# sanowl/CUDA-NT-Xent-MPI-NCCL-SimCLR

Hardware: AMD Instinct MI355X
Metric: NT-Xent fwd+bwd samples/sec, B=4096 d=2048, at 1/2/4/8 MI355X (higher is better)
Workload: dtype bf16

## Files before the change

cuda-nt-xent-mpi-nccl-simclr_amd/csrc/kernels/ntxent_kernels.hip:

```cpp

#include "../include/ntxent/ntxent.h"
#include "device_common.h"
#include "sim_gemm.h"

#include <atomic>
#include <algorithm>
#include <cmath>
#include <cstdio>
#include <cstdlib>
#include <mutex>
#include <string>
#include <type_traits>
#include <vector>
#include <unordered_map>

namespace ntxent {
namespace dev {

template <typename T> __device__ __forceinline__ void load8(const T* p, float (&v)[8]);
template <> __device__ __forceinline__ void load8<float>(const float* p, float (&v)[8]) {
  const f32x4 a = *reinterpret_cast<const f32x4*>(p), b = *reinterpret_cast<const f32x4*>(p + 4);
  v[0] = a[0]; v[1] = a[1]; v[2] = a[2]; v[3] = a[3]; v[4] = b[0]; v[5] = b[1]; v[6] = b[2]; v[7] = b[3];
}
template <typename T> __device__ __forceinline__ void load8_h(const T* p, float (&v)[8]) {
// ... 1457 lines not shown
  NTXENT_HIP_CHECK(hipGetLastError());
}

int dot_slots(const Geometry& g) { return 4 * g.col_tiles; }

void launch_dot_reduce(const float* dotp, float* dot, const Geometry& g, hipStream_t stream) {
  hipLaunchKernelGGL(dev::dot_reduce_kernel, dim3((g.rows_pad + 31) / 32), dim3(256), 0, stream, dotp, dot_slots(g),
                     g.rows_pad, dot);
  NTXENT_HIP_CHECK(hipGetLastError());
}

static bool apply_norm_fuse(dev::SimParams& p, const NormFuse* nf, const Geometry& g) {
  if (nf == nullptr || nf->dh == nullptr || g.dim % 8 != 0) return false;
  p.nh = nf->h;
  p.nh_dt = nf->in == DType::F32 ? 0 : (nf->in == DType::F16 ? 1 : 2);
  p.nd = g.dim;
  p.ninv = nf->inv;
  p.ndot = nf->dot;
  p.ngo = nf->grad_out;
  p.nalpha = (float)(1.0 / ((double)g.global_rows * g.temperature));
  p.ndh = nf->dh;
  p.out_f16 = 1;
  p.accum = 0;
  return true;
}

bool launch_dz(DType comp, const void* sc, const void* zqt_all, const int4* tiles, int ntiles,
               void* slabs, const GemmWorkspace& ws, const Geometry& g, hipStream_t stream, bool out_f16,
               const NormFuse* nf, const Q8Stats* q8, const float* cpos, bool half_c) {
  if (ntiles == 0) return false;
  NTXENT_CHECK(!half_c || dz_half_c_eligible(comp, g, ntiles, ws), "dz: half C not eligible for this launch");
  const bool f8 = comp == DType::FP8;
  NTXENT_CHECK(!f8 || (q8 && q8->mneg2 && q8->lmin && q8->zq && cpos && g.world == 1 && out_f16),
               "dz (fp8 backward): Q8Stats, cpos, world 1 and an fp16 slab required");
  const long long cs = (long long)dtype_size(comp);
  dev::SimParams p = base_params(g);
  if (f8) {
    p.q8_mneg = q8->mneg2;
    p.q8_lmin = q8->lmin;
    p.q8_zq = static_cast<const _Float16*>(q8->zq);
    p.q8_ldz = g.ld_k;
    p.cpos = cpos;
  }
  p.A = coef_tile_operand(sc, g.col_tiles, cs);
  p.B.base = static_cast<const char*>(zqt_all);
  const long long ldt = f8 ? q8_ldt(g) : g.ld_t;
  p.B.ld = ldt * cs;
  p.B.row_tile_stride = (long long)kTile * ldt * cs;
  p.B.kblk = (long long)g.rows_pad * cs;
  p.B.kblk_stride = (long long)g.dim_n * ldt * cs;
  p.tiles = tiles;
  p.kbytes = (long long)g.world * g.rows_pad * cs;
  p.out = static_cast<float*>(slabs);
  p.out_f16 = out_f16 ? 1 : 0;
  p.ldo = g.dim_n;
  p.slab_stride = (long long)g.rows_pad * g.dim_n;
  const int cus = ws.sched_cus > 0 ? std::min(ws.sched_cus, ws.num_cus) : ws.num_cus;
  const int nk = (int)(p.kbytes / kKStepBytes);
  int pieces = fwd_splitk_pieces(ntiles, nk, cus, 1);
  if (pieces < 3 || f8) pieces = 0;
  int grid;
  if (pieces > 0) {
    p.nk = nk;
    p.dp_tiles = 0;
    p.sk_tiles = ntiles;
    p.ipb = (nk + pieces - 1) / pieces;
    p.sk_cnt = static_cast<int*>(ws.ptr);
    p.sk_slabs = reinterpret_cast<float*>(static_cast<char*>(ws.ptr) + sk_counter_bytes(ws.num_cus));
    p.splitk = 1;
    grid = (int)((nk + p.ipb - 1) / p.ipb) * ntiles;
    NTXENT_CHECK(p.kbytes % kKStepBytes == 0 && grid <= ws.num_cus && ws.ptr != nullptr &&
                     ws.bytes >= gemm_workspace_bytes(ntiles, ws.num_cus),
                 "split-K dZ: workspace too small");
  } else {
    grid = apply_schedule(p, ntiles, ws, stream);
  }
  if (half_c)
    NTXENT_CHECK(((pieces == 0 && p.sk_tiles == 0 && p.dp_tiles == ntiles) || (pieces > 0 && p.ipb % 2 == 0)) &&
                     (long long)g.row_tiles * g.col_tiles * kTileElems * cs < (1ll << 31),
                 "dz: half C needs items starting at even K-steps and a C buffer below 2 GiB (32-bit offsets)");
  p.c_half = half_c ? 1 : 0;
  const bool fused = comp != DType::F32 && apply_norm_fuse(p, nf, g);
  if (fused) NTXENT_CHECK(nf->dot != nullptr, "dz: fused normalisation backward without dot");
  if (nf && nf->dot_cnt) {
    NTXENT_CHECK(fused && !f8 && nf->dotp && dz_dot_fold_eligible(comp, g, ntiles, ws),
                 "dz: dot fold needs the fused 16-bit epilogue");
    p.dotp = const_cast<float*>(nf->dotp);
    p.dot_nslot = dot_slots(g);
    p.dot_cnt = pieces == 0 ? nf->dot_cnt : nullptr;
    p.dot_spin = dot_fold_spin();
  }
  dispatch_gemm(comp, [&](auto tc) {
    using Tc = decltype(tc);
    launch_sim_gemm<Tc, dev::kModeDz>(grid, p, stream);
  });
  if (pieces > 0) hipLaunchKernelGGL(dev::sk_dz_reduce_kernel, dim3(ntiles * 64), dim3(256), 0, stream, p);
  NTXENT_HIP_CHECK(hipGetLastError());
  return fused;
}

void launch_dz_view(DType comp, const void* a, long long a_panel_tiles, const void* b, long long b_kblk_cols,
                    long long b_kblk_stride, int k_tiles, const int4* tiles, int ntiles, void* out, bool accum,
                    const GemmWorkspace& ws, const Geometry& g, hipStream_t stream, bool out_f16) {
  NTXENT_CHECK(!(accum && out_f16), "dz_view: fp16 output cannot accumulate");
  if (ntiles == 0 || k_tiles == 0) return;
  NTXENT_CHECK(k_tiles > 0 && a_panel_tiles >= k_tiles, "dz_view: bad K extent");
  const long long cs = (long long)dtype_size(comp);
  dev::SimParams p = base_params(g);
  p.A = coef_tile_operand(a, a_panel_tiles, cs);
  NTXENT_CHECK(b_kblk_cols > 0 && b_kblk_cols % kTile == 0, "dz_view: bad B K block");
  p.B.base = static_cast<const char*>(b);
  p.B.ld = (long long)g.ld_t * cs;
  p.B.row_tile_stride = (long long)kTile * g.ld_t * cs;
  p.B.kblk = b_kblk_cols * cs;
  p.B.kblk_stride = b_kblk_stride * cs;
  p.tiles = tiles;
  p.kbytes = (long long)k_tiles * kTile * cs;
  p.out = static_cast<float*>(out);
  p.ldo = g.dim_n;
  p.slab_stride = (long long)g.rows_pad * g.dim_n;
  p.accum = accum ? 1 : 0;
  p.out_f16 = out_f16 ? 1 : 0;
  const int grid = apply_schedule(p, ntiles, ws, stream);
  dispatch_comp(comp, [&](auto tc) {
    using Tc = decltype(tc);
    launch_sim_gemm<Tc, dev::kModeDz>(grid, p, stream);
  });
  NTXENT_HIP_CHECK(hipGetLastError());
}

void launch_norm_bwd(DType in, const float* slabs, int nslabs, const void* h, const float* inv,
                     const float* grad_out, void* dh, const Geometry& g, hipStream_t stream,
                     const void* xslabs, int nx) {
  const _Float16* xs = static_cast<const _Float16*>(xslabs);
  if (xs == nullptr) nx = 0;
  const float alpha_base = (float)(1.0 / ((double)g.global_rows * g.temperature));
  const long long ss = (long long)g.rows_pad * g.dim_n, ldo = g.dim_n;
  const int nch = (g.dim + 2047) / 2048;
  const bool vec = (g.dim % 8) == 0 && nch <= 4;
  dispatch_comp(in, [&](auto tin) {
    using Tin = decltype(tin);
    const Tin* hp = static_cast<const Tin*>(h);
    Tin* dp = static_cast<Tin*>(dh);
    if (vec && nch == 1)
      hipLaunchKernelGGL((dev::norm_bwd_vec_kernel<Tin, 1>), dim3(g.rows), dim3(256), 0, stream, slabs, nslabs, ss,
                         ldo, hp, inv, grad_out, alpha_base, dp, g.dim, xs, nx);
    else if (vec && nch == 2)
      hipLaunchKernelGGL((dev::norm_bwd_vec_kernel<Tin, 2>), dim3(g.rows), dim3(256), 0, stream, slabs, nslabs, ss,
                         ldo, hp, inv, grad_out, alpha_base, dp, g.dim, xs, nx);
    else if (vec)
      hipLaunchKernelGGL((dev::norm_bwd_vec_kernel<Tin, 4>), dim3(g.rows), dim3(256), 0, stream, slabs, nslabs, ss,
                         ldo, hp, inv, grad_out, alpha_base, dp, g.dim, xs, nx);
    else
      hipLaunchKernelGGL((dev::norm_bwd_kernel<Tin>), dim3(g.rows), dim3(256), 0, stream, slabs, nslabs, ss, ldo,
                         hp, inv, grad_out, alpha_base, dp, g.dim, xs, nx);
  });
  NTXENT_HIP_CHECK(hipGetLastError());
}

const DeviceInfo& device_info(int device) {
  static std::mutex mu;
  static std::unordered_map<int, DeviceInfo> cache;
  std::lock_guard<std::mutex> lock(mu);
  auto it = cache.find(device);
  if (it != cache.end()) return it->second;
  hipDeviceProp_t prop;
// ... 23 lines not shown
```

cuda-nt-xent-mpi-nccl-simclr_amd/csrc/kernels/sim_gemm.h:

```cpp
#pragma once

#include "../include/ntxent/ntxent.h"
#include "device_common.h"

#include <type_traits>

namespace ntxent {
namespace dev {

enum SimMode : int { kModeFwd = 0, kModeCoef = 1, kModeDz = 2 };

constexpr int kStageBytes = 2 * kTile * kKStepBytes;
#ifndef NTXENT_GEMM_DMA_AUX
#define NTXENT_GEMM_DMA_AUX 0
#endif
constexpr int kGemmDmaAux = NTXENT_GEMM_DMA_AUX;
#ifndef NTXENT_TIMING
#define NTXENT_TIMING 0
#endif
constexpr int kTimingItems = 8;
constexpr int kTimingMarks = 8;
__device__ __forceinline__ void store16_wt(void* base, long long off, u32x4 v) {
  const unsigned lo = __builtin_amdgcn_readfirstlane((unsigned)off);
  const unsigned hi = __builtin_amdgcn_readfirstlane((unsigned)((unsigned long long)off >> 32));
// ... 75 lines not shown

__device__ __forceinline__ int sc_unit(int rb, int cb, int lane) { return ((rb >> 4) * 8 + (cb >> 5)) * 64 + lane; }

struct KStream {
  const char* ptr;
  int kin, left;
  int kk;
  __device__ __forceinline__ void init(const char* base, long long k0, const OperandDesc& o, int nk) {
    kin = (int)(k0 % o.kblk);
    ptr = base + (k0 / o.kblk) * o.kblk_stride + kin;
    left = nk - 1;
    kk = (int)(k0 / kKStepBytes);
  }
  __device__ __forceinline__ void advance(const OperandDesc& o) {
    if (left > 0) {
      --left;
      ++kk;
      ptr += kKStepBytes;
      kin += kKStepBytes;
      if (kin == (int)o.kblk) { kin = 0; ptr += o.kblk_stride - o.kblk; }
    }
  }
  __device__ __forceinline__ void skip() {
    if (left > 0) {
      --left;
      ++kk;
    }
  }
  __device__ __forceinline__ void seek(const char* base, long long k0, const OperandDesc& o) {
    kin = (int)(k0 % o.kblk);
    ptr = base + (k0 / o.kblk) * o.kblk_stride + kin;
  }
};

__device__ __forceinline__ int ct_swz(int L) {
  return ((L >> 1) & 1) | ((L & 1) << 1) | (((L >> 3) & 1) << 2) | ((((L >> 1) ^ (L >> 2)) & 1) << 3);
}

__device__ __forceinline__ void dot_slot_store(float* p, float v) { *p = v; }

__device__ __forceinline__ long long ctile_index(const SimParams& p, int mt, int nt) {
  const int cs = p.c_rot ? (nt - p.row_tile0 + p.col_tiles) % p.col_tiles : nt - p.c_tile0;
  return (long long)mt * p.c_ld + cs;
}

template <typename T, int NW, int NMI = 8>
__device__ __forceinline__ void coef_epilogue(f32x4 (&acc)[NMI][4], const int (&rb)[NMI], const int (&cb)[4],
                                              int row_base, int col_base, int mt, int nt, int kind,
                                              lds_char* lds, const SimParams& p, int lane) {
  constexpr int NROWS = NW == 8 ? kTile : NMI * 16;
  constexpr int NCOLS = NW == 8 ? kTile : 64;
#ifndef NTXENT_COEF_SWZ
#define NTXENT_COEF_SWZ 1
#endif
  constexpr bool SWZ = NW == 1 && NTXENT_COEF_SWZ;
  static_assert(!SWZ || (NROWS == 64 && NCOLS == 64), "swizzled C^T staging is for 64 x 64 regions");
  constexpr int S = SWZ ? 128 : NROWS * 2 + 16;
  auto ct_at = [&](int L, int e) { return SWZ ? L * S + (((e >> 2) ^ ct_swz(L)) << 3) : L * S + e * 2; };
  constexpr int NT = NW * 64;
  T* base = reinterpret_cast<T*>(p.cbuf);
  const int col_local0 = (nt * kTile) % p.Rpad;
  const bool fixed = p.fixed_shift != 0;
  const float M = p.y_scale;
  float lcol[4];
  bool cvalid[4];
  int gj[4];
#pragma unroll
  for (int ni = 0; ni < 4; ++ni) {
    const int col_t = cb[ni] + (lane & 15);
    gj[ni] = nt * kTile + col_t;
    const float l = p.lse2[gj[ni]];
    lcol[ni] = fixed ? fast_exp2(M - l) : l;
    cvalid[ni] = (col_local0 + col_t) < p.R;
  }
  T* slot = base + ctile_index(p, mt, nt) * kTileElems;
  T* mirror = nullptr;
  if ((kind == kTileSymOff && !p.c_half) || kind == kTileDiagUp)
    mirror = base + ctile_index(p, nt - p.row_tile0, p.row_tile0 + mt) * kTileElems;
  else if (kind == kTileCross) {
    const int rt = p.Rpad / kTile, W = p.col_tiles / rt, q = nt / rt;
    const int slot = (q - p.row_tile0 / rt - 1 + W) % W;
    mirror = reinterpret_cast<T*>(p.mbuf) + ((long long)(slot * rt + nt % rt) * rt + mt) * kTileElems;
  }
  const int wq = NW == 8 ? ((threadIdx.x >> 6) & 3) : (col_base >> 6);
  float cdot[2][4] = {{0.f, 0.f, 0.f, 0.f}, {0.f, 0.f, 0.f, 0.f}};
  const int r_lo = mt * kTile + row_base, r_hi = r_lo + NROWS;
  const int c_lo = nt * kTile + col_base, c_hi = c_lo + NCOLS;
  auto hits = [&](int a0) { return a0 < c_hi && c_lo < a0 + NROWS; };
  const bool plain = fixed && r_hi <= p.R && col_local0 + col_base + NCOLS <= p.R && !hits(p.own0 + r_lo) &&
                     !hits(p.own0 + r_lo + p.n_half) && !hits(p.own0 + r_lo - p.n_half);
#pragma unroll
  for (int mi = 0; mi < NMI; ++mi) {
    float c[4][4];
    const int row_t0 = rb[mi] + 4 * (lane >> 4);
    const int gi0 = mt * kTile + row_t0;
    const f32x4 lrow4 = *reinterpret_cast<const f32x4*>(p.lse2 + p.own0 + gi0);
    const f32x4 cpos4 = *reinterpret_cast<const f32x4*>(p.cpos + gi0);
    if (plain) {
#pragma unroll
      for (int r = 0; r < 4; ++r) {
        const float lrow = fast_exp2(M - lrow4[r]);
#pragma unroll
        for (int ni = 0; ni < 4; ++ni) c[ni][r] = fast_exp2(acc[mi][ni][r] * p.acc_scale - M) * (lrow + lcol[ni]);
      }
    } else
#pragma unroll
    for (int r = 0; r < 4; ++r) {
      const int gi = gi0 + r;
      const bool rvalid = gi < p.R;
      const float lrow = fixed ? fast_exp2(M - lrow4[r]) : lrow4[r];
      const int gself = p.own0 + gi;
      const int gpos = p.own0 + (gi < p.n_half ? gi + p.n_half : gi - p.n_half);
#pragma unroll
      for (int ni = 0; ni < 4; ++ni) {
        const float y = acc[mi][ni][r] * p.acc_scale;
        float v = fixed ? fast_exp2(y - M) * (lrow + lcol[ni]) : fast_exp2(y - lrow) + fast_exp2(y - lcol[ni]);
        v = (gj[ni] == gpos) ? cpos4[r] : v;
        v = (rvalid && cvalid[ni] && gj[ni] != gself) ? v : 0.0f;
        c[ni][r] = v;
      }
    }
    if (p.dotp) {
#pragma unroll
      for (int r = 0; r < 4; ++r) {
        float d = 0.f;
#pragma unroll
        for (int ni = 0; ni < 4; ++ni) d += to_f32<T>(from_f32<T>(c[ni][r])) * acc[mi][ni][r];
        d = row16_sum(d);
        const int row = mt * kTile + rb[mi] + 4 * (lane >> 4) + r;
        if ((lane & 15) == 0) dot_slot_store(p.dotp + (long long)(nt * 4 + wq) * p.Rpad + row, d);
      }
      const int h2 = NMI == 8 ? (mi >> 2) : 0;
#pragma unroll
      for (int ni = 0; ni < 4; ++ni)
#pragma unroll
        for (int r = 0; r < 4; ++r) cdot[h2][ni] += to_f32<T>(from_f32<T>(c[ni][r])) * acc[mi][ni][r];
    }
#pragma unroll
    for (int ni = 0; ni < 4; ++ni) {
      const int col_t = cb[ni] + (lane & 15);
      if constexpr (sizeof(T) == 2) {
        union { T h[4]; u32x2 u; } pk;
#pragma unroll
        for (int r = 0; r < 4; ++r) pk.h[r] = from_f32<T>(c[ni][r]);
        *reinterpret_cast<__attribute__((address_space(3))) u32x2*>(lds + ct_at(col_t - col_base, row_t0 - row_base)) =
            pk.u;
      } else {
#pragma unroll
        for (int r = 0; r < 4; ++r)
          *reinterpret_cast<float*>(reinterpret_cast<char*>(slot) + ctile_off(row_t0 + r, col_t, 4)) = c[ni][r];
        if (mirror)
          *reinterpret_cast<f32x4*>(reinterpret_cast<char*>(mirror) + ctile_off(col_t, row_t0, 4)) =
              f32x4{c[ni][0], c[ni][1], c[ni][2], c[ni][3]};
      }
    }
  }
  if (p.dotp) {
    if (kind == kTileSymOff || kind == kTileDiagUp) {
      const int wa8 = (threadIdx.x >> 6) >> 2;
#pragma unroll
      for (int h2 = 0; h2 < (NMI == 8 ? 2 : 1); ++h2)
#pragma unroll
        for (int ni = 0; ni < 4; ++ni) {
          const float d = xrow_sum(cdot[h2][ni]);
          const int rq = NMI == 8 ? 2 * h2 + wa8 : (row_base >> 6);
          const int row = (nt - p.row_tile0) * kTile + cb[ni] + (lane & 15);
          if (lane < 16) dot_slot_store(p.dotp + (long long)((p.row_tile0 + mt) * 4 + rq) * p.Rpad + row, d);
        }
    }
  }
  if constexpr (sizeof(T) == 2) {
    __syncthreads();
    const int tid = threadIdx.x, w = tid >> 6;
    if (mirror) {
      constexpr int CPR = NROWS * 2 / 16;
#pragma unroll 4
      for (int q = 0; q < NCOLS * CPR / NT; ++q) {
        const int k = tid + NT * q;
        const int row = k / CPR, c16 = k % CPR;
        u32x4 v;
        if constexpr (SWZ) {
          typedef __attribute__((address_space(3))) const u32x2 lds_u2;
          const u32x2 lo = *(lds_u2*)(lds + ct_at(row, 8 * c16)), hi = *(lds_u2*)(lds + ct_at(row, 8 * c16 + 4));
          v = u32x4{lo[0], lo[1], hi[0], hi[1]};
        } else {
          v = *reinterpret_cast<const __attribute__((address_space(3))) u32x4*>(lds + row * S + c16 * 16);
        }
        *reinterpret_cast<u32x4*>(reinterpret_cast<char*>(mirror) + ctile_off(col_base + row, row_base + 8 * c16, 2)) = v;
      }
    }
    typedef short v4s __attribute__((ext_vector_type(4)));
    constexpr int RB = NROWS / 16;
    constexpr int NBLK = RB * (NCOLS / 32) / NW;
    const int g = lane >> 4, i = lane & 15, q4 = i >> 2, p4 = i & 3;
#pragma unroll 2
    for (int b = 0; b < NBLK; ++b) {
      const int blk = w * NBLK + b;
      const int c0 = (blk % RB) * 16;
      const int r0 = (blk / RB) * 32 + 8 * g;
      const lds_char* a0 = lds + ct_at(r0 + q4, c0 + 4 * p4);
      const lds_char* a1 = lds + ct_at(r0 + q4 + 4, c0 + 4 * p4);
      const v4s lo = __builtin_amdgcn_ds_read_tr16_b64_v4i16((__attribute__((address_space(3))) v4s*)a0);
      const v4s hi = __builtin_amdgcn_ds_read_tr16_b64_v4i16((__attribute__((address_space(3))) v4s*)a1);
      u32x4 u;
      u[0] = (unsigned short)lo[0] | ((unsigned)(unsigned short)lo[1] << 16);
      u[1] = (unsigned short)lo[2] | ((unsigned)(unsigned short)lo[3] << 16);
      u[2] = (unsigned short)hi[0] | ((unsigned)(unsigned short)hi[1] << 16);
      u[3] = (unsigned short)hi[2] | ((unsigned)(unsigned short)hi[3] << 16);
      const int src = ((lane >> 2) + 16 * (lane & 3)) << 2;
      u32x4 v;
#pragma unroll
      for (int k = 0; k < 4; ++k) v[k] = (unsigned)__builtin_amdgcn_ds_bpermute(src, (int)u[k]);
      char* cdst = reinterpret_cast<char*>(slot) +
                   ctile_off(row_base + c0 + (lane >> 2), col_base + (blk / RB) * 32 + 8 * (lane & 3), 2);
#ifndef NTXENT_COEF_STORE
#define NTXENT_COEF_STORE 0
#endif
      if constexpr (NTXENT_COEF_STORE == 1)
        __builtin_nontemporal_store(v, reinterpret_cast<u32x4*>(cdst));
      else if constexpr (NTXENT_COEF_STORE == 2)
        store16_wt(slot, cdst - reinterpret_cast<char*>(slot), v);
      else
        *reinterpret_cast<u32x4*>(cdst) = v;
    }
  }
}

__device__ __forceinline__ unsigned q8_pack4(float x0, float x1, float x2, float x3) {
  const int w = __builtin_amdgcn_cvt_pk_fp8_f32(fminf(x0, 448.f), fminf(x1, 448.f), 0, false);
  return (unsigned)__builtin_amdgcn_cvt_pk_fp8_f32(fminf(x2, 448.f), fminf(x3, 448.f), w, true);
}
__device__ __forceinline__ float q8_dot4(unsigned w, const f32x4& a) {
  typedef float f2 __attribute__((ext_vector_type(2)));
  const f2 lo = __builtin_amdgcn_cvt_pk_f32_fp8((int)w, false), hi = __builtin_amdgcn_cvt_pk_f32_fp8((int)w, true);
  return fmaf(lo[0], a[0], fmaf(lo[1], a[1], fmaf(hi[0], a[2], hi[1] * a[3])));
}

template <typename TS>
__device__ __forceinline__ void coef_epilogue_q8(f32x4 (&acc)[4][4], const int (&rb)[4], const int (&cb)[4],
                                                 int row_base, int col_base, int mt, int nt, int kind, lds_char* lds,
                                                 const SimParams& p, int lane) {
  constexpr int S8 = 80;
  lds_char* ld_d = lds;
  lds_char* ld_m = lds + 64 * S8;
  unsigned char* base = reinterpret_cast<unsigned char*>(p.cbuf);
  unsigned char* slot = base + ctile_index(p, mt, nt) * kTileElems;
  const bool mirrored = kind == kTileSymOff || kind == kTileDiagUp;
  unsigned char* mirror = mirrored ? base + ctile_index(p, nt - p.row_tile0, p.row_tile0 + mt) * kTileElems : nullptr;
  const int col_local0 = (nt * kTile) % p.Rpad;
  const bool fixed = p.fixed_shift != 0;
  const float M = p.y_scale;
  const float lmin = p.q8_lmin[0];
  float lcol[4], scol[4], icol[4];
  bool cvalid[4];
  int gj[4];
#pragma unroll
// ... 251 lines not shown
  int k = sg;
  for (; k + 120 < nslot; k += 128) {
    float v[16];
#pragma unroll
    for (int u = 0; u < 16; ++u) v[u] = dotp[(long long)(k + 8 * u) * rows + i];
#pragma unroll
    for (int u = 0; u < 16; ++u) s += v[u];
  }
  for (; k < nslot; k += 8) s += dotp[(long long)k * rows + i];
  return s;
}

__device__ __forceinline__ void dz_dot_fold(const SimParams& p, lds_char* lds, int tid) {
  typedef __attribute__((address_space(3))) float lds_fl;
  lds_fl* part = (lds_fl*)lds;
  const int G = gridDim.x, rows = p.Rpad;
  const int rpb = ((rows + G - 1) / G + 31) & ~31;
  const int r0 = blockIdx.x * rpb, r1 = r0 + rpb < rows ? r0 + rpb : rows;
  const int hf = tid >> 8, lt = tid & 255, ln = lt & 63, sg = 2 * (lt >> 6) + (ln >> 5);
  const auto drs = __builtin_amdgcn_make_buffer_rsrc(const_cast<float*>(p.ndot), 0, 0x7FFFFFFF, 0x00020000);
  for (int c0 = r0; c0 < r1; c0 += 64) {
    const int i = c0 + 32 * hf + (ln & 31);
    part[(hf * 8 + sg) * 32 + (ln & 31)] = i < r1 ? dot_slot_sum(p.dotp, p.dot_nslot, rows, i, sg) : 0.f;
    __syncthreads();
    if (lt < 32 && c0 + 32 * hf + lt < r1) {
      float t = 0.f;
#pragma unroll
      for (int g = 0; g < 8; ++g) t += part[(hf * 8 + g) * 32 + lt];
      __builtin_amdgcn_raw_buffer_store_b32(__float_as_uint(t), drs, (c0 + 32 * hf + lt) * 4, 0, 16);
    }
    __syncthreads();
  }
}
template <bool FOLD>
__device__ __forceinline__ float dz_dot(const SimParams& p, int row, int& state) {
  if (!FOLD || p.dot_cnt == nullptr) return p.ndot[row];
  if (state == 0) {
    int n = 0;
    bool done = false;
    while (!(done = __hip_atomic_load(p.dot_cnt, __ATOMIC_RELAXED, __HIP_MEMORY_SCOPE_AGENT) >= (int)gridDim.x) &&
           n < p.dot_spin) {
      __builtin_amdgcn_s_sleep(8);
      ++n;
    }
    state = done && p.dot_spin > 0 ? 1 : 2;
  }
  if (state == 2) {
    float t = 0.f;
    for (int g = 0; g < 8; ++g) {
      float s = 0.f;
      for (int k = g; k < p.dot_nslot; k += 8) s += p.dotp[(long long)k * p.Rpad + row];
      t += s;
    }
    return t;
  }
  const auto drs = __builtin_amdgcn_make_buffer_rsrc(const_cast<float*>(p.ndot), 0, 0x7FFFFFFF, 0x00020000);
  return __uint_as_float(__builtin_amdgcn_raw_buffer_load_b32(drs, row * 4, 0, 16));
}
__device__ __forceinline__ void dz_dot_exit(const SimParams& p, int tid, bool counted) {
  if (!counted) asm volatile("s_waitcnt vmcnt(0)" ::: "memory");
  __syncthreads();
  if (tid == 0) {
    if (!counted) __hip_atomic_fetch_add(p.dot_cnt, 1, __ATOMIC_RELAXED, __HIP_MEMORY_SCOPE_AGENT);
    const int old = __hip_atomic_fetch_add(p.dot_cnt + 1, 1, __ATOMIC_RELAXED, __HIP_MEMORY_SCOPE_AGENT);
    if (old == (int)gridDim.x - 1) {
      __hip_atomic_store(p.dot_cnt, 0, __ATOMIC_RELAXED, __HIP_MEMORY_SCOPE_AGENT);
      __hip_atomic_store(p.dot_cnt + 1, 0, __ATOMIC_RELAXED, __HIP_MEMORY_SCOPE_AGENT);
    }
  }
}

__device__ __forceinline__ constexpr int hpiece_lds(int i) {
  return i == 0 ? 0 : i == 1 ? kStageBytes : i == 2 ? kStageBytes + kHalfBytes : i == 3 ? kHalfBytes
       : i == 4 ? kTile * kKStepBytes : i == 5 ? kStageBytes + kTile * kKStepBytes
       : i == 6 ? kStageBytes + kTile * kKStepBytes + kHalfBytes : kGemmLds + 2048;
}
constexpr int kHPieceExtra = 16384;

__device__ __forceinline__ void dz_store_h(f32x4 (&acc)[8][4], const SimParams& p, int mt, int nt, int tid,
                                           const int (&rb)[8], const int (&cb)[4], lds_char* lds, float iv0, float dt0) {
  typedef __attribute__((address_space(3))) u32x2 lds_u2;
  typedef __attribute__((address_space(3))) u32x4 lds_u4;
  typedef __attribute__((address_space(3))) f32x2 lds_f2;
  const int lane = tid & 63, wb = (tid >> 6) & 3;
  const float sgo = p.ngo[0] * p.nalpha;
  lds_f2* cf = (lds_f2*)(lds + kTile * 512);
  if (tid < kTile) cf[tid] = f32x2{sgo * iv0, sgo * iv0 * iv0 * dt0};
  asm volatile("s_waitcnt vmcnt(0)" ::: "memory");
  __syncthreads();
  const bool bf = p.nh_dt == 2;
#pragma unroll
  for (int mi = 0; mi < 8; ++mi) {
    const int r = (rb[mi] & 127) + (lane & 15);
    const f32x2 c = cf[rb[mi] + (lane & 15)];
    const int rofs = r * kKStepBytes;
    const int sw = (r >> 1) & 7;
#pragma unroll
    for (int ni = 0; ni < 4; ++ni) {
      const int nn = (cb[ni] + 4 * (lane >> 4)) & 63;
      const int a = (wb >> 1) ? hpiece_lds(4 * (ni >> 1) + 2 + (mi >> 2)) : hpiece_lds(4 * (ni >> 1) + (mi >> 2));
      lds_u2* hp = (lds_u2*)(lds + a + rofs + (((nn >> 3) ^ sw) << 4) + ((nn & 7) << 1));
      union { _Float16 f[4]; __bf16 b[4]; u32x2 u; } x, y;
      x.u = *hp;
#pragma unroll
      for (int e = 0; e < 4; ++e) {
        const float g = (float)(_Float16)acc[mi][ni][e];
        const float hv = bf ? (float)x.b[e] : (float)x.f[e];
        const float o = c.x * g - c.y * hv;
        if (bf) y.b[e] = (__bf16)o;
        else y.f[e] = (_Float16)o;
      }
      *hp = y.u;
    }
  }
  __syncthreads();
  const long long nd = p.nd;
#pragma unroll
  for (int k = 0; k < 16; ++k) {
    const int i = k >> 1, r = (tid >> 3) + 64 * (k & 1), c = tid & 7;
    const u32x4 v = *(lds_u4*)(lds + hpiece_lds(i) + r * kKStepBytes + ((c ^ ((r >> 1) & 7)) << 4));
    const long long m = (long long)mt * kTile + 128 * (i & 1) + r;
    store16_wt(p.ndh, (m * nd + nt * kTile + 64 * (i >> 1) + 8 * c) * 2, v);
  }
}

template <typename T>
__device__ __forceinline__ void dz_store(f32x4 (&acc)[8][4], const SimParams& p, int mt, int nt, int tid,
                                         const int (&rb)[8], const int (&cb)[4], lds_char* lds, int& dstate) {
  constexpr bool kFold = !std::is_same<T, fp8e4m3>::value && sizeof(T) == 2;
  typedef __attribute__((address_space(3))) u32x4 lds_u4;
  const int lane = tid & 63;
  float* out = p.out;
  if (p.out_f16 && !p.accum) {
    typedef __attribute__((address_space(3))) u32x2 lds_u2;
    float iv0 = 0.f, dt0 = 0.f;
    if (p.ndh && tid < kTile && mt * kTile + tid < p.R) {
      iv0 = p.ninv[mt * kTile + tid];
      dt0 = dz_dot<kFold>(p, mt * kTile + tid, dstate);
    }
#pragma unroll
    for (int mi = 0; mi < 8; ++mi) {
      const int rt = rb[mi] + (lane & 15);
#pragma unroll
      for (int ni = 0; ni < 4; ++ni) {
        const int ct = cb[ni] + 4 * (lane >> 4);
        union { _Float16 h[4]; u32x2 u; } pk;
#pragma unroll
        for (int r = 0; r < 4; ++r) pk.h[r] = (_Float16)acc[mi][ni][r];
        *(lds_u2*)(lds + rt * 512 + ((((ct >> 3) ^ (rt & 15))) << 4) + ((ct >> 2) & 1) * 8) = pk.u;
      }
    }
    const bool h16 = p.ndh && p.nh_dt != 0;
    u32x4 hq[16];
    if (h16) {
#pragma unroll
      for (int k = 0; k < 16; ++k) {
        const int idx = tid + kGemmThreads * k, rt = idx >> 5, c = idx & 31;
        const int m = mt * kTile + rt, d0 = nt * kTile + 8 * c;
        hq[k] = (m < p.R && d0 < p.nd)
                    ? *reinterpret_cast<const u32x4*>(static_cast<const char*>(p.nh) + ((long long)m * p.nd + d0) * 2)
                    : u32x4{0u, 0u, 0u, 0u};
      }
    }
    __syncthreads();
    if (p.ndh) {
      const float sgo = p.ngo[0] * p.nalpha;
      typedef __attribute__((address_space(3))) float lds_fl;
      lds_fl* cf = (lds_fl*)(lds + kTile * 512);
      if (tid < kTile) {
        cf[2 * tid] = sgo * iv0;
        cf[2 * tid + 1] = sgo * iv0 * iv0 * dt0;
      }
      __syncthreads();
#pragma unroll
      for (int k = 0; k < 16; ++k) {
        const int idx = tid + kGemmThreads * k, rt = idx >> 5, c = idx & 31;
        const int m = mt * kTile + rt, d0 = nt * kTile + 8 * c;
        if (m >= p.R || d0 >= p.nd) continue;
        union { _Float16 h[8]; u32x4 u; } g;
        g.u = *(lds_u4*)(lds + rt * 512 + ((c ^ (rt & 15)) << 4));
        const float c1 = cf[2 * rt], c2 = cf[2 * rt + 1];
        const long long off = (long long)m * p.nd + d0;
        float hv[8], o[8];
        if (p.nh_dt == 2) {
          union { __bf16 h[8]; u32x4 u; } x;
          x.u = hq[k];
#pragma unroll
          for (int e = 0; e < 8; ++e) hv[e] = (float)x.h[e];
        } else if (p.nh_dt == 1) {
          union { _Float16 h[8]; u32x4 u; } x;
          x.u = hq[k];
#pragma unroll
          for (int e = 0; e < 8; ++e) hv[e] = (float)x.h[e];
        } else {
          const f32x4* hp = reinterpret_cast<const f32x4*>(static_cast<const float*>(p.nh) + off);
          const f32x4 a = hp[0], b = hp[1];
#pragma unroll
          for (int e = 0; e < 4; ++e) { hv[e] = a[e]; hv[4 + e] = b[e]; }
        }
#pragma unroll
        for (int e = 0; e < 8; ++e) o[e] = c1 * (float)g.h[e] - c2 * hv[e];
        if (p.nh_dt == 2) {
          union { __bf16 h[8]; u32x4 u; } y;
#pragma unroll
          for (int e = 0; e < 8; ++e) y.h[e] = (__bf16)o[e];
          store16_wt(p.ndh, off * 2, y.u);
// ... 274 lines not shown
      tr_base = p.A.base + (long long)tt.x * p.A.kblk_stride;
      tr_end = p.c_half ? 4 * tt.x : 0;
    }
    const int ns = ke - kb;
    const char* Ab = p.A.base + (long long)tt.x * p.A.row_tile_stride;
    const char* Bb = p.B.base + (long long)(tt.y - p.b_tile0) * p.B.row_tile_stride;
    const long long k0 = (long long)kb * kKStepBytes;
    sa0.init(Ab, k0, p.A, ns); sa1.init(Ab, k0, p.A, ns);
    if constexpr (kTrCap) {
      if (tr_end > kb) {
        sa0.seek(Ab, (long long)tr_end * kKStepBytes, p.A);
        sa1.seek(Ab, (long long)tr_end * kKStepBytes, p.A);
      }
    }
    sb0.init(Bb, k0, p.B, ns); sb1.init(Bb, k0, p.B, ns);
    if constexpr (kF8 && MODE != kModeDz) {
      const int t = threadIdx.x;
      const char* src = (t < 256 ? Ab + (long long)t * p.A.ld : Bb + (long long)(t - 256) * p.B.ld) + p.scale_off;
      __builtin_amdgcn_global_load_lds((const void*)src, (lds_void*)(lds + kScaleLds + 256 * w), 4, 0, 0);
    }
    stage(0, 0, sa0, 0); stage(1, 0, sb0, 0); stage(1, 1, sb1, 0); stage(0, 1, sa1, 0);
    stage(0, 0, sa0, 1); stage(1, 0, sb0, 1); stage(1, 1, sb1, 1);
  };
  const bool streaming = kStreamMode && p.sk_tiles == 0 && nk >= 2 && (nk & 1) == 0;
  bool streamed = false;
  int dstate = 0;
  bool dot_counted = false;
  if constexpr (MODE == kModeDz && !kF8 && sizeof(T) == 2) {
    if (p.dot_nslot > 0) dz_dot_fold(p, lds + kGemmLds, threadIdx.x);
  }
  auto tmark = [&](int item, int k) {
#if NTXENT_TIMING
    if (threadIdx.x == 0 && item < kTimingItems)
      p.tstamp[((long long)blockIdx.x * kTimingItems + item) * kTimingMarks + k] = __builtin_amdgcn_s_memtime();
#endif
  };
  for (int item = 0;; ++item) {
  tmark(item, 0);
  int tile, kb, ke, stile;
  if (streamed) {
    tile = bid + item * G; kb = 0; ke = nk; stile = -1;
  } else {
    if (!fetch(item, tile, kb, ke, stile)) break;
    prologue(tile, kb, ke, item & 1);
  }
  const bool cont = streaming && item + 1 < n_dp;
  const char* na = nullptr;
  const char* nb = nullptr;
  int nmt = 0, nnt = 0;
  if (cont) {
    const int4 tn = sload_int4(p.tiles, bid + (item + 1) * G);
    na = p.A.base + (long long)tn.x * p.A.row_tile_stride;
    nb = p.B.base + (long long)(tn.y - p.b_tile0) * p.B.row_tile_stride;
    nmt = tn.x;
    nnt = tn.y;
  }
  const int4 t = sload_int4(p.tiles, tile);
  const int mt = t.x, nt = t.y;
  const int nsteps = ke - kb;
#pragma unroll
  for (int mi = 0; mi < 8; ++mi)
#pragma unroll
    for (int ni = 0; ni < 4; ++ni) acc[mi][ni] = f32x4{0.f, 0.f, 0.f, 0.f};

  asm volatile("s_waitcnt vmcnt(10)" ::: "memory");
  barrier();
  if constexpr (MODE == kModeDz && !kF8 && sizeof(T) == 2) {
    if (item == 0 && p.dot_cnt != nullptr && threadIdx.x == 0)
      __hip_atomic_fetch_add(p.dot_cnt, 1, __ATOMIC_RELAXED, __HIP_MEMORY_SCOPE_AGENT);
    dot_counted = true;
  }
  if constexpr (kF8 && MODE != kModeDz) {
    const int r16_ = lane & 15;
    unsigned av[8], bv[4];
    lds_get_scales((unsigned)(uintptr_t)(lds + kScaleLds) + 4 * (64 * wa + r16_),
                   (unsigned)(uintptr_t)(lds + kScaleLds) + 4 * (256 + 32 * wb + r16_), av, bv);
    sa_v[0] = pack_low_bytes(av[0], av[1], av[2], av[3]);
    sa_v[1] = pack_low_bytes(av[4], av[5], av[6], av[7]);
    sb_v = pack_low_bytes(bv[0], bv[1], bv[2], bv[3]);
  }
  tmark(item, 1);
  if (grp == 1) barrier();
  bool hpre = false;
  if constexpr (MODE == kModeDz && !kF8)
    hpre = p.ndh != nullptr && (p.nh_dt == 1 || p.nh_dt == 2) && stile < 0 && nsteps == nk && nsteps >= 4 &&
           (nsteps & 1) == 0 && p.R % kTile == 0 && p.nd % kTile == 0;
  auto kstep = [&](const int ks, auto cur_c, auto tail_c, auto tr_c) {
    constexpr int cur = decltype(cur_c)::value, nxt = cur ^ 1;
    constexpr int TAIL = decltype(tail_c)::value;
    constexpr bool TR = decltype(tr_c)::value != 0;
    constexpr int TRM = decltype(tr_c)::value == 0 ? 0 : (decltype(tr_c)::value == 2 ? 1 : 2);
    if constexpr (kStreamMode) {
      if (cont && ks == nsteps - 2) {
        sa0.init(na, 0, p.A, nk); sb0.init(nb, 0, p.B, nk); sb1.init(nb, 0, p.B, nk);
        if (p.inv_a) stage_inv(nmt, nnt, (item + 1) & 1);
      }
      if (cont && ks == nsteps - 1) sa1.init(na, 0, p.A, nk);
    }
    dma_wait(); barrier();
    if constexpr (TR) read_a_tr(cur_c, kI0, af);
    else read_a(cur, 0, af);
    __builtin_amdgcn_sched_barrier(0);
    read_b(cur, 0, bf0);
    if constexpr (TAIL == 2) stage_h(3, mt, nt);
    else stage(0, 1, sa1, nxt, TRM);
    a0_retire(); barrier();
    lds_drain();
    if constexpr (TR) __builtin_amdgcn_sched_barrier(0);
    mma_quadrant(kI0, kI0, af, bf0);
    dma_wait(); barrier();
    read_b(cur, 1, bf1);
    if constexpr (TAIL != 0) stage_h(TAIL == 1 ? 0 : 4, mt, nt);
    else stage(0, 0, sa0, cur, TRM);
    barrier(); lds_drain();
    mma_quadrant(kI0, kI1, af, bf1);
    barrier();
    if constexpr (TR) read_a_tr(cur_c, kI1, af);
    else read_a(cur, 1, af);
    if constexpr (TAIL != 0) stage_h(TAIL == 1 ? 1 : 5, mt, nt);
    else stage(1, 0, sb0, cur);
    barrier(); lds_drain();
    if constexpr (TR) __builtin_amdgcn_sched_barrier(0);
    mma_quadrant(kI1, kI0, af, bf0);
    if constexpr (TAIL != 2) dma_wait();
    barrier();
    if constexpr (TAIL != 0) {
      stage_h(TAIL == 1 ? 2 : 6, mt, nt);
      if constexpr (TAIL == 2) stage_h(7, mt, nt);
    } else {
      stage(1, 1, sb1, cur);
    }
    barrier();
    mma_quadrant(kI1, kI1, af, bf1);
  };
  const std::integral_constant<int, 2> kI2{};
  int ks2 = 0;
  const int nmain = nsteps - (hpre ? 2 : 0);
  if constexpr (kTrCap) {
    const int ntr = tr_end > kb ? (tr_end < ke ? tr_end : ke) - kb : 0;
    for (; ks2 + 3 < ntr; ks2 += 2) {
      kstep(ks2, kI0, kI0, kI1);
      kstep(ks2 + 1, kI1, kI0, kI1);
    }
    if (ks2 + 1 < ntr) {
      kstep(ks2, kI0, kI0, kI2);
      kstep(ks2 + 1, kI1, kI0, kI2);
      ks2 += 2;
    }
  }
  for (; ks2 + 1 < nmain; ks2 += 2) {
    kstep(ks2, kI0, kI0, kI0);
    kstep(ks2 + 1, kI1, kI0, kI0);
  }
  if constexpr (MODE == kModeDz && !kF8) {
    if (hpre) {
      kstep(ks2, kI0, kI1, kI0);
      kstep(ks2 + 1, kI1, kI2, kI0);
      ks2 += 2;
    }
  }
  if (ks2 < nsteps) kstep(ks2, kI0, kI0, kI0);
  if (grp == 0) barrier();
  tmark(item, 2);
  float hiv = 0.f, hdt = 0.f;
  if constexpr (MODE == kModeDz && !kF8) {
    if (hpre && threadIdx.x < kTile) {
      hiv = p.ninv[mt * kTile + threadIdx.x];
// ... 900 lines not shown
```

Before: 11.23 million.

## Write coef tiles row-major via DPP shuffle and pipeline fused dh epilogue stores

In the coefficient epilogue, non-mirrored tiles now pair lanes with a DPP swap and byte permute so the LDS staging is row-major, then copy out with contiguous 16-byte row stores and return early. The fused normalisation-backward dz epilogue is restructured into two row halves: each half is formed in LDS, then stored with buffer stores that use a scalar base resource and 32-bit offsets. This lets the first half's global writes overlap forming the second half and takes per-store address math off the vector units. A new size check enforces the 32-bit offset limit, and the dh prefetch path is restricted to 16-bit types.

```diff
diff --git a/cuda-nt-xent-mpi-nccl-simclr_amd/csrc/kernels/ntxent_kernels.hip b/cuda-nt-xent-mpi-nccl-simclr_amd/csrc/kernels/ntxent_kernels.hip
--- a/cuda-nt-xent-mpi-nccl-simclr_amd/csrc/kernels/ntxent_kernels.hip
+++ b/cuda-nt-xent-mpi-nccl-simclr_amd/csrc/kernels/ntxent_kernels.hip
@@ -1563,6 +1563,7 @@
   p.c_half = half_c ? 1 : 0;
   const bool fused = comp != DType::F32 && apply_norm_fuse(p, nf, g);
   if (fused) NTXENT_CHECK(nf->dot != nullptr, "dz: fused normalisation backward without dot");
+  if (fused) NTXENT_CHECK((long long)kTile * g.dim * 2 < (1ll << 31), "dz: 256 rows of dh must stay below 2 GiB");
   if (nf && nf->dot_cnt) {
     NTXENT_CHECK(fused && !f8 && nf->dotp && dz_dot_fold_eligible(comp, g, ntiles, ws),
                  "dz: dot fold needs the fused 16-bit epilogue");
diff --git a/cuda-nt-xent-mpi-nccl-simclr_amd/csrc/kernels/sim_gemm.h b/cuda-nt-xent-mpi-nccl-simclr_amd/csrc/kernels/sim_gemm.h
--- a/cuda-nt-xent-mpi-nccl-simclr_amd/csrc/kernels/sim_gemm.h
+++ b/cuda-nt-xent-mpi-nccl-simclr_amd/csrc/kernels/sim_gemm.h
@@ -181,6 +181,16 @@
     const int slot = (q - p.row_tile0 / rt - 1 + W) % W;
     mirror = reinterpret_cast<T*>(p.mbuf) + ((long long)(slot * rt + nt % rt) * rt + mt) * kTileElems;
   }
+#ifndef NTXENT_COEF_ROWMAJOR
+#define NTXENT_COEF_ROWMAJOR 1
+#endif
+  const bool direct = SWZ && NTXENT_COEF_ROWMAJOR && mirror == nullptr;
+  const int odd = lane & 1;
+  const unsigned psel0 = odd ? 0x01000504u : 0x05040100u, psel1 = odd ? 0x03020706u : 0x07060302u;
+  auto rm_at = [&](int ni) {
+    const int g4 = lane >> 4, jj = (lane >> 3) & 1, dw = (lane >> 1) & 3;
+    return (4 * g4 + 2 * odd) * 128 + ((2 * (ni ^ ((2 * g4 + odd) & 3)) + jj) << 4) + dw * 4;
+  };
   const int wq = NW == 8 ? ((threadIdx.x >> 6) & 3) : (col_base >> 6);
   float cdot[2][4] = {{0.f, 0.f, 0.f, 0.f}, {0.f, 0.f, 0.f, 0.f}};
   const int r_lo = mt * kTile + row_base, r_hi = r_lo + NROWS;
@@ -242,6 +252,14 @@
         union { T h[4]; u32x2 u; } pk;
 #pragma unroll
         for (int r = 0; r < 4; ++r) pk.h[r] = from_f32<T>(c[ni][r]);
+        if (direct) {
+          typedef __attribute__((address_space(3))) unsigned lds_u1;
+          const unsigned send = odd ? pk.u[0] : pk.u[1], keep = odd ? pk.u[1] : pk.u[0];
+          const unsigned recv = (unsigned)__builtin_amdgcn_mov_dpp((int)send, 0xB1, 0xF, 0xF, true);
+          lds_u1* d = (lds_u1*)(lds + rm_at(ni) + 16 * mi * 128);
+          d[0] = __builtin_amdgcn_perm(recv, keep, psel0);
+          d[32] = __builtin_amdgcn_perm(recv, keep, psel1);
+        } else
         *reinterpret_cast<__attribute__((address_space(3))) u32x2*>(lds + ct_at(col_t - col_base, row_t0 - row_base)) =
             pk.u;
       } else {
@@ -271,6 +289,18 @@
   if constexpr (sizeof(T) == 2) {
     __syncthreads();
     const int tid = threadIdx.x, w = tid >> 6;
+    if (direct) {
+      typedef __attribute__((address_space(3))) const u32x4 lds_u4;
+      const int rr = lane >> 3, ch = lane & 7;
+      const lds_char* src = lds + rr * 128 + ((ch ^ (((rr >> 1) & 3) << 1)) << 4);
+      char* cdst = reinterpret_cast<char*>(slot) + ctile_off(row_base + rr, col_base + 8 * ch, 2);
+#pragma unroll
+      for (int b = 0; b < 8; ++b) {
+        const u32x4 v = *(lds_u4*)(src + b * 1024);
+        *reinterpret_cast<u32x4*>(cdst + ctile_off(8 * b, 0, 2)) = v;
+      }
+      return;
+    }
     if (mirror) {
       constexpr int CPR = NROWS * 2 / 16;
 #pragma unroll 4
@@ -688,46 +718,77 @@
   typedef __attribute__((address_space(3))) u32x2 lds_u2;
   typedef __attribute__((address_space(3))) u32x4 lds_u4;
   typedef __attribute__((address_space(3))) f32x2 lds_f2;
-  const int lane = tid & 63, wb = (tid >> 6) & 3;
+  const int lane = tid & 63;
+  const int wb = __builtin_amdgcn_readfirstlane(tid >> 6) & 3;
   const float sgo = p.ngo[0] * p.nalpha;
   lds_f2* cf = (lds_f2*)(lds + kTile * 512);
   if (tid < kTile) cf[tid] = f32x2{sgo * iv0, sgo * iv0 * iv0 * dt0};
   asm volatile("s_waitcnt vmcnt(0)" ::: "memory");
   __syncthreads();
+  const int ch0 = (4 * (wb & 1) + (lane >> 5)) ^ ((lane >> 1) & 7);
+  const int lrow = ((rb[0] & 127) + (lane & 15)) * kKStepBytes + (((lane >> 4) & 1) << 3);
+  const int loff[2] = {lrow + (ch0 << 4), lrow + ((ch0 ^ 2) << 4)};
+  int nd_e = p.nd;
+  char* dh_e = static_cast<char*>(p.ndh);
+  asm volatile("" : "+s"(nd_e), "+s"(dh_e));
+  const long long nd = nd_e;
+  const auto hrs = __builtin_amdgcn_make_buffer_rsrc(
+      dh_e + ((long long)mt * kTile * nd + (long long)nt * kTile) * 2, 0, 0x7FFFFFFF, 0x00020000);
+  const int ndb = nd_e * 2;
+  const int st_v = (tid >> 3) * ndb + ((tid & 7) << 4);
+  const int st_l = (tid >> 3) * kKStepBytes + (((tid & 7) ^ ((tid >> 4) & 7)) << 4);
   const bool bf = p.nh_dt == 2;
-#pragma unroll
-  for (int mi = 0; mi < 8; ++mi) {
-    const int r = (rb[mi] & 127) + (lane & 15);
-    const f32x2 c = cf[rb[mi] + (lane & 15)];
-    const int rofs = r * kKStepBytes;
-    const int sw = (r >> 1) & 7;
-#pragma unroll
-    for (int ni = 0; ni < 4; ++ni) {
-      const int nn = (cb[ni] + 4 * (lane >> 4)) & 63;
-      const int a = (wb >> 1) ? hpiece_lds(4 * (ni >> 1) + 2 + (mi >> 2)) : hpiece_lds(4 * (ni >> 1) + (mi >> 2));
-      lds_u2* hp = (lds_u2*)(lds + a + rofs + (((nn >> 3) ^ sw) << 4) + ((nn & 7) << 1));
-      union { _Float16 f[4]; __bf16 b[4]; u32x2 u; } x, y;
-      x.u = *hp;
-#pragma unroll
-      for (int e = 0; e < 4; ++e) {
-        const float g = (float)(_Float16)acc[mi][ni][e];
-        const float hv = bf ? (float)x.b[e] : (float)x.f[e];
-        const float o = c.x * g - c.y * hv;
-        if (bf) y.b[e] = (__bf16)o;
-        else y.f[e] = (_Float16)o;
-      }
-      *hp = y.u;
-    }
-  }
-  __syncthreads();
-  const long long nd = p.nd;
-#pragma unroll
-  for (int k = 0; k < 16; ++k) {
-    const int i = k >> 1, r = (tid >> 3) + 64 * (k & 1), c = tid & 7;
-    const u32x4 v = *(lds_u4*)(lds + hpiece_lds(i) + r * kKStepBytes + ((c ^ ((r >> 1) & 7)) << 4));
-    const long long m = (long long)mt * kTile + 128 * (i & 1) + r;
-    store16_wt(p.ndh, (m * nd + nt * kTile + 64 * (i >> 1) + 8 * c) * 2, v);
-  }
+  auto form = [&](auto rh_c) {
+    constexpr int rh = decltype(rh_c)::value;
+#pragma unroll
+    for (int nh = 0; nh < 2; ++nh) {
+      const int a = (wb >> 1) ? hpiece_lds(4 * nh + 2 + rh) : hpiece_lds(4 * nh + rh);
+#pragma unroll
+      for (int q = 0; q < 2; ++q) {
+        lds_char* hb = lds + a + loff[q];
+#pragma unroll
+        for (int m3 = 0; m3 < 4; ++m3) {
+          const int mi = 4 * rh + m3, ni = 2 * nh + q;
+          const f32x2 c = cf[rb[mi] + (lane & 15)];
+          lds_u2* hp = (lds_u2*)(hb + m3 * 16 * kKStepBytes);
+          union { _Float16 f[4]; __bf16 b[4]; u32x2 u; } x, y;
+          x.u = *hp;
+#pragma unroll
+          for (int e = 0; e < 4; ++e) {
+            const float g = (float)(_Float16)acc[mi][ni][e];
+            const float hv = bf ? (float)x.b[e] : (float)x.f[e];
+            const float o = c.x * g - c.y * hv;
+            if (bf) y.b[e] = (__bf16)o;
+            else y.f[e] = (_Float16)o;
+          }
+          *hp = y.u;
+        }
+      }
+    }
+  };
+  auto store = [&](auto rh_c) {
+    constexpr int rh = decltype(rh_c)::value;
+    u32x4 v[8];
+#pragma unroll
+    for (int k = 0; k < 8; ++k)
+      v[k] = *(lds_u4*)(lds + hpiece_lds(2 * (k >> 1) + rh) + st_l + (k & 1) * 64 * kKStepBytes);
+#pragma unroll
+    for (int k = 0; k < 8; ++k)
+      __builtin_amdgcn_raw_buffer_store_b128(v[k], hrs, st_v + 128 * (k >> 1), (128 * rh + 64 * (k & 1)) * ndb, 16);
+  };
+  const std::integral_constant<int, 0> k0{};
+  const std::integral_constant<int, 1> k1{};
+  auto lds_barrier = [&]() {
+    asm volatile("s_waitcnt lgkmcnt(0)" ::: "memory");
+    __builtin_amdgcn_s_barrier();
+    asm volatile("" ::: "memory");
+  };
+  form(k0);
+  lds_barrier();
+  store(k0);
+  form(k1);
+  lds_barrier();
+  store(k1);
 }
 
 template <typename T>
@@ -1168,7 +1229,7 @@
   tmark(item, 1);
   if (grp == 1) barrier();
   bool hpre = false;
-  if constexpr (MODE == kModeDz && !kF8)
+  if constexpr (MODE == kModeDz && !kF8 && sizeof(T) == 2)
     hpre = p.ndh != nullptr && (p.nh_dt == 1 || p.nh_dt == 2) && stile < 0 && nsteps == nk && nsteps >= 4 &&
            (nsteps & 1) == 0 && p.R % kTile == 0 && p.nd % kTile == 0;
   auto kstep = [&](const int ks, auto cur_c, auto tail_c, auto tr_c) {
```

Result: no change. 11.21 million (-0.2%).
